# jzombie/rust-llkv

Hardware: NVIDIA B200
Metric: tpch_q6_lineitem_rows_per_sec (higher is better)
Workload: dtype i128/i64 (Decimal128, Date32)

## Files before the change

### rust-llkv_b200/csrc/compiler.cpp

```cpp
#include "compiler.h"

#include <algorithm>

#include <math.h>
#include <stdarg.h>
#include <stdio.h>
#include <stdlib.h>
#include <string.h>

#include <map>
#include <stdexcept>

namespace llkv {

typedef __int128 i128;
typedef unsigned __int128 u128;

namespace {

struct CompileError {
  int32_t code;
  std::string msg;
};

// ... 1683 lines not shown
    out_.fast = false;
    p.n_finstr = 0;
    if (!req_.no_fast) {
      const size_t lits_mark = lits_.size();
      if (lower_fast()) {
        out_.fast = true;
        bool checked = false;
        for (uint32_t i = 0; i < p.n_finstr; ++i) {
          const FInstr& fi = p.fcode[i];
          const uint32_t fb = fi.a & 0x7f;
          if ((fi.op == FO_OP_COL || fi.op == FO_OP_LIT || fi.op == FO_OP_TMP) && (fb == FB_ADD_CK || fb == FB_SUB_CK || fb == FB_MUL_CK)) checked = true;
        }
        out_.can_narrow_fail = checked;
        p.n_lits = (uint32_t)lits_.size();
        for (size_t i = 0; i < lits_.size(); ++i) p.lits[i] = lits_[i];
      } else {
        lits_.resize(lits_mark);
        p.n_finstr = 0;
      }
    }
  }

  struct Iv {
    bool known = false;
    i128 lo = 0, hi = 0;
    bool is_float = false;
  };
  static Iv iv_exact(i128 v) {
    Iv x;
    x.known = true;
// ... 66 lines not shown
    else if (verbose) fprintf(stderr, "[llkv] lean lowering gave up at compiler.cpp:%d\n", line);
    return false;
  }
  bool lower_fast() {
    Plan& p = out_.plan;
    if (wide_ || req_.bitmap_mode) return lf_fail(__LINE__);
    if (plan_cols_.empty()) return lf_fail(__LINE__);
    for (const ColumnMeta* c : plan_cols_) {
      if (c->load_kind == LK_D128 && !c->dec_fits_i64) return lf_fail(__LINE__);
    }
    std::vector<FInstr> f;
    std::vector<Sym> st;
    bool tmp_used[kFastTmps] = {false, false, false};
    int max_tmps = 0;
    bool ok = true;
    auto map_load = [&](uint8_t lk) -> uint32_t {
      switch (lk) {
        case LK_I32: case LK_D32: return LKF_4;
        case LK_I64: case LK_U64: case LK_F64: case LK_D64: return LKF_8;
        case LK_D128: return LKF_16;
        case LK_U8: return LKF_1;
        case LK_STR8: return LKF_S1;
        case LK_I8: return LKF_1S;
        case LK_I16: return LKF_2;
        case LK_U16: return LKF_2U;
        case LK_U32: return LKF_4U;
        case LK_F32: return LKF_4F;
        default: ok = false; return LKF_8;
      }
    };
    auto femit = [&](uint16_t op, uint32_t a, uint32_t b, uint32_t c) {
// ... 30 lines not shown
        if (i == keep || st[i].where != Sym::ACC) continue;
        int k = -1;
        for (int t = 0; t < kFastTmps; ++t)
          if (!tmp_used[t]) { k = t; break; }
        if (k < 0) { ok = false; return; }
        tmp_used[k] = true;
        if (k + 1 > max_tmps) max_tmps = k + 1;
        femit(FO_ST_TMP, (uint8_t)k, 0, 0);
        st[i].where = Sym::TMP;
        st[i].tmp = (uint8_t)k;
      }
    };
    auto load_acc = [&](size_t i) {
      if (st[i].where == Sym::ACC) return;
      spill_acc(i);
      if (st[i].where == Sym::COL) femit_load(FO_LD_COL, 2, st[i].col, map_load(st[i].load));
      else if (st[i].where == Sym::LIT) femit_load(FO_LD_LIT, 1, st[i].lit, 0);
      else {
        femit_load(FO_LD_TMP, 3, st[i].tmp, 0);
        tmp_used[st[i].tmp] = false;
      }
      st[i].where = Sym::ACC;
    };
    auto emit_binary = [&](uint8_t fb) {
      const size_t n = st.size();
      Sym& a = st[n - 2];
      Sym& b = st[n - 1];
      uint8_t rev = 0;
      const Sym* other;
      if (a.where == Sym::ACC) other = &b;
      else if (b.where == Sym::ACC) { other = &a; rev = FB_REV; }
      else { load_acc(n - 2); other = &b; }
      if (!ok) return;
      if (other->where == Sym::COL) femit(FO_OP_COL, fb | rev, map_load(other->load), other->col);
      else if (other->where == Sym::LIT) femit(FO_OP_LIT, fb | rev, 0, other->lit);
      else femit(FO_OP_TMP, fb | rev, other->tmp, 0);
      free_sym(*other);
    };
    auto fold_lit = [&](Sym& x, i128 v) {
      x.lit = add_lit((uint64_t)(u128)v, (uint64_t)((u128)v >> 64));
      x.iv = iv_exact(v);
    };

    if (p.n_fast_words > (uint32_t)kLeanMaxWords) return lf_fail(__LINE__);
    for (uint32_t w = 0; w < p.n_fast_words; ++w) p.fast[w].lean_width = p.fast[w].lean_rowrel = 0;
    auto lean_word = [&](uint32_t w, uint8_t width, bool rowrel) {
      if (w >= p.n_fast_words) { ok = false; return; }
      if (p.fast[w].lean_width && (p.fast[w].lean_rowrel != 0) != rowrel) width = 8, rowrel = false;
      if (width > p.fast[w].lean_width) p.fast[w].lean_width = width;
// ... 40 lines not shown
                  }
                  continue;
                }
                if (pr.op == OP_IN_D) {
                  const i128 v = (i128)(((u128)L.hi << 64) | (u128)L.lo);
                  if (!fits_i64(v)) {
                    if (c.load_kind == LK_D128) return lf_fail(__LINE__);
                    continue;
                  }
                }
                run.push_back(mk_lit_i((i128)(int64_t)L.lo));
              }
              if (c.load_kind == LK_D128 && !c.dec_fits_i64) return lf_fail(__LINE__);
              if (lits_.size() + run.size() + 1 > (size_t)kMaxLits) return lf_fail(__LINE__);
              const uint32_t first = run.empty() ? 0u : add_lit_run(run);
              femit(FO_LEAF, in.a, map_load(in.b), first);
              f.back().g = 3u;
              f.back().f = (uint32_t)run.size();
              f.back().e = push;
              i += conjunct ? 2 : 1;
              break;
            }
            if (pr.op == OP_PRED_F) {
              const bool f32 = c.load_kind == LK_F32;
              auto key = [&](double d) -> int64_t {
                if (f32) {
                  const float x = (float)d;
                  int32_t b;
                  memcpy(&b, &x, 4);
                  return (int64_t)(b ^ ((b >> 31) & INT32_MAX));
                }
// ... 74 lines not shown
                  if (uk != LLKV_BOUND_UNBOUNDED) {
                    const i128 v = lit_val(li);
                    if (uk == LLKV_BOUND_EXCLUDED) { if (v <= tmin) empty = true; else hi = v - 1; } else hi = v;
                  }
                }
                if (lo < tmin) lo = tmin;
                if (hi > tmax) hi = tmax;
                if (lo > hi) empty = true;
              }
              Lit a, b;
              if (empty) { a = mk_lit_i(1); b = mk_lit_i(0); }
              else { a = mk_lit_i(lo); b = mk_lit_i(hi); }
              std::vector<Lit> run = {a, b};
              if (lits_.size() + 2 > (size_t)kMaxLits) return lf_fail(__LINE__);
              const uint32_t first = add_lit_run(run);
              femit(FO_LEAF, in.a, map_load(in.b), first);
              f.back().g = uns ? 1u : 0u;
              if (c.load_kind == LK_STR8 || c.load_kind == LK_U8 || c.load_kind == LK_U64) f.back().g = 1u;
              f.back().e = push;
              i += conjunct ? 2 : 1;
              break;
            }
          }
          Sym x;
          x.where = Sym::COL;
          x.col = in.a;
          x.load = in.b;
          x.iv = column_interval(c);
          x.nm = c.nullable ? (1u << in.a) : 0u;
          st.push_back(x);
          break;
// ... 101 lines not shown
          const size_t n2 = st.size();
          uint32_t cmp = in.a;
          const Sym* other;
          if (st[n2 - 2].where == Sym::ACC) other = &st[n2 - 1];
          else if (st[n2 - 1].where == Sym::ACC) {
            static const uint8_t mirrored[6] = {LLKV_CMP_EQ, LLKV_CMP_NE, LLKV_CMP_GT, LLKV_CMP_GE, LLKV_CMP_LT, LLKV_CMP_LE};
            other = &st[n2 - 2];
            cmp = mirrored[cmp];
          } else {
            load_acc(n2 - 2);
            other = &st[n2 - 1];
          }
          if (!ok) return lf_fail(__LINE__);
          const uint32_t kind = in.op == OP_CMP_U ? 1u : in.op == OP_CMP_F ? 2u : 0u;
          const uint32_t nm = st[n2 - 1].nm | st[n2 - 2].nm;
          if (other->where == Sym::COL) femit(FO_CMP, cmp | (kind << 4), 0u | (map_load(other->load) << 8), other->col);
          else if (other->where == Sym::LIT) femit(FO_CMP, cmp | (kind << 4), 1u, other->lit);
          else femit(FO_CMP, cmp | (kind << 4), 2u, other->tmp);
          f.back().h = nm;
          free_sym(st[n2 - 1]);
          free_sym(st[n2 - 2]);
          st.pop_back();
          st.pop_back();
          ++mask_depth;
          break;
        }
        case OP_ISNULL: {
          if (i >= select_end_ || st.empty() || mask_depth >= 8) return lf_fail(__LINE__);
          const uint32_t nm = st.back().nm;
          free_sym(st.back());
          st.pop_back();
// ... 20 lines not shown
          if (mask_depth != 1) return lf_fail(__LINE__);
          femit(FO_MASK_FILTER, 0, 0, 0);
          mask_depth = 0;
          break;
        case OP_MVCC: femit(FO_MVCC, in.a, in.b, 0); break;
        case OP_SELECT_DONE: femit(FO_SELECT_DONE, 0, 0, 0); break;
        case OP_GROUP: {
          const int nk = in.a;
          if ((int)st.size() < nk) return lf_fail(__LINE__);
          for (int k = nk - 1; k >= 0; --k) {
            const Sym x = st.back();
            if (x.where != Sym::COL) return lf_fail(__LINE__);
            if (x.nm && (p.single_wide_key || !p.key_nullable[k])) return lf_fail(__LINE__);
            st.pop_back();
            p.key_col[k] = x.col;
            p.key_load[k] = (uint8_t)map_load(x.load);
          }
          femit(FO_GROUP, (uint8_t)nk, 0, 0);
          break;
        }
        case OP_AGG_COUNT_STAR: femit(FO_COUNT_STAR, 0, in.b, in.c); lean_word(in.b, 4, false); break;
        case OP_AGG_FIRSTROW: femit(FO_FIRSTROW, 0, in.b, in.c); lean_word(in.b, 4, true); break;
        case OP_AGG_COUNT: case OP_AGG_SUM_I: case OP_AGG_SUM_D: case OP_AGG_FSUM: case OP_AGG_MIN_I: case OP_AGG_MAX_I:
        case OP_AGG_MIN_F: case OP_AGG_MAX_F: case OP_AGG_FIRSTVALID: case OP_AGG_FIRSTNAN: case OP_AGG_MIN_D: case OP_AGG_MAX_D: {
          if (st.empty()) return lf_fail(__LINE__);
          uint8_t a = 0;
          uint16_t op;
          bool keep = (in.a & 1) != 0;
          uint8_t width = 8;
          bool rowrel = false;
          switch (in.op) {
// ... 101 lines not shown
```

### rust-llkv_b200/csrc/compiler.h

```cpp
#pragma once
#include <stdint.h>

#include <string>
#include <vector>

#include "../../include/llkv_gpu.h"
#include "plan.h"

namespace llkv {

struct ColumnMeta {
  uint64_t field_id = 0;
  int32_t type = 0;
  int precision = 0, scale = 0;
  bool nullable = false;
  uint8_t load_kind = 0;
  uint32_t elem_bytes = 0;
  uint32_t arrow_bytes = 0;
  const void* dev_values = nullptr;
  const unsigned char* dev_validity = nullptr;
  uint64_t n_rows = 0;
  bool dec_fits_i64 = true;
  uint64_t min_bits = 0, max_bits = 0;
  bool has_minmax = false;
  uint8_t max_strlen = 0;
  bool str_non_ascii = false;
  const std::vector<std::string>* dict_sorted = nullptr;
  uint64_t dict_epoch = 0;
};

inline void literal_bytes(const llkv_literal& l, const char** p, size_t* n) {
  if (l.precision == LLKV_LIT_STRING_BY_REF) {
    *p = reinterpret_cast<const char*>(static_cast<uintptr_t>(l.lo));
    *n = static_cast<size_t>(l.hi);
  } else {
// ... 86 lines not shown
```

### rust-llkv_b200/csrc/lean_kernel.cuh

```cuda
#pragma once
#include "device_util.cuh"
#include "plan.h"

namespace llkv {

#define LLKV_FULL 0xffffffffu
#define LLKV_SLOW_HERE (SLOW && has_slow)

__device__ __forceinline__ double lean_f64(i64 v) { return __longlong_as_double(v); }
__device__ __forceinline__ i64 lean_bits(double d) { return __double_as_longlong(d); }

constexpr u64 kSlotTableFull = 1ull << 63;
static __device__ __noinline__ u64 lean_global_slot_raw(u64* gkeys, u64 gcap, uint32_t n_keys, u64 K) {
  if (n_keys == 0) return 0;
  if (K == kEmptyKey) return gcap;
  const u64 mask = gcap - 1;
  u64 h = mix64(K) & mask;
  for (u64 i = 0; i <= mask; ++i) {
    u64 cur = gkeys[h];
    if (cur == K) return h;
    if (cur == kEmptyKey) {
      const u64 old = atomicCAS(&gkeys[h], kEmptyKey, K);
      if (old == kEmptyKey || old == K) return h;
    }
// ... 370 lines not shown
          } else {
            const u64 span = (u64)hi - (u64)lo;
#pragma unroll
            for (int r = 0; r < R; ++r) {
              const i64 b = reinterpret_cast<const i64*>(base)[r * NC + tid];
              m |= (unsigned)(((u64)(b ^ ((b >> 63) & 0x7fffffffffffffffll)) - (u64)lo) <= span) << r;
            }
          }
        } else if (in.b == LKF_4) {
          const uint32_t l = (uint32_t)(int)lo, span = (uint32_t)(int)hi - l;
#pragma unroll
          for (int r = 0; r < R; ++r) {
            const uint32_t v = reinterpret_cast<const uint32_t*>(base)[r * NC + tid];
            m |= (unsigned)((v - l) <= span) << r;
          }
        } else if ((in.b == LKF_8 || in.b == LKF_16) && in.g == 0) {
          const u64 span = (u64)hi - (u64)lo;
          const int stride = in.b == LKF_16 ? 2 : 1;
#pragma unroll
          for (int r = 0; r < R; ++r) {
            const u64 v = reinterpret_cast<const u64*>(base)[stride * (r * NC + tid)];
            m |= (unsigned)((v - (u64)lo) <= span) << r;
          }
        } else {
          i64 v[R];
          load_col(in.a, in.b, v);
          const u64 span = (u64)hi - (u64)lo;
#pragma unroll
          for (int r = 0; r < R; ++r) m |= (unsigned)(((u64)v[r] - (u64)lo) <= span) << r;
        }
// ... 999 lines not shown
```

### rust-llkv_b200/csrc/llkv_gpu.cu

```cuda
#include <cuda_runtime.h>
#include <dlfcn.h>
#include <math.h>
#include <stdarg.h>
#include <stdio.h>
#include <stdlib.h>
#include <string.h>

#include <algorithm>
#include <atomic>
#include <map>
#include <memory>
#include <mutex>
#include <string>
#include <deque>
#include <string_view>
#include <thread>
#include <unordered_map>
#include <vector>

#include "../../include/llkv_gpu.h"
#include "compiler.h"
#include "jit.h"
#include "plan.h"
#include "upload.h"
// ... 170 lines not shown
  for (u64 i = (u64)blockIdx.x * blockDim.x + threadIdx.x; i < n; i += (u64)gridDim.x * blockDim.x) {
    const ulonglong2 w = in[i];
    out[i] = w.x;
    b = b || (i64)w.y != ((i64)w.x >> 63);
  }
  if (b) atomicOr(bad, 1u);
}
__global__ void narrow_dec32_kernel(const ulonglong2* __restrict__ in, int* __restrict__ out, u64 n) {
  for (u64 i = (u64)blockIdx.x * blockDim.x + threadIdx.x; i < n; i += (u64)gridDim.x * blockDim.x) out[i] = (int)in[i].x;
}
__global__ void widen_dec32_kernel(const int* __restrict__ in, ulonglong2* __restrict__ out, u64 n) {
  for (u64 i = (u64)blockIdx.x * blockDim.x + threadIdx.x; i < n; i += (u64)gridDim.x * blockDim.x) {
    const i64 v = in[i];
    out[i] = make_ulonglong2((u64)v, (u64)(v >> 63));
  }
}
__global__ void widen_dec_kernel(const u64* __restrict__ in, ulonglong2* __restrict__ out, u64 n) {
  for (u64 i = (u64)blockIdx.x * blockDim.x + threadIdx.x; i < n; i += (u64)gridDim.x * blockDim.x) {
    const u64 v = in[i];
    out[i] = make_ulonglong2(v, (u64)((i64)v >> 63));
  }
}
__global__ void widen_str_kernel(const unsigned char* __restrict__ in, u64* __restrict__ out, u64 n) {
  for (u64 i = (u64)blockIdx.x * blockDim.x + threadIdx.x; i < n; i += (u64)gridDim.x * blockDim.x) out[i] = ((u64)in[i] << 56) | 1ull;
}
__global__ void or_bits_kernel(unsigned int* __restrict__ dst, u64 dst_off, const unsigned char* __restrict__ src, u64 n) {
  const u64 nw = (n + 31) / 32;
  for (u64 w = (u64)blockIdx.x * blockDim.x + threadIdx.x; w < nw; w += (u64)gridDim.x * blockDim.x) {
    unsigned int bits = 0;
    for (int b = 0; b < 4; ++b) {
// ... 476 lines not shown
  std::vector<NarrowChunk> narrow_chunks;
  uint64_t h2d_bytes = 0;
  unsigned int* d_perm = nullptr;
  uint64_t perm_chunk_rows = 0, perm_version = 0;
  bool sparse = false;
  void* pend_dst = nullptr;
  const void* pend_src = nullptr;
  uint64_t pend_bytes = 0;
  std::vector<void*> deferred_free;
  uint64_t version = 1;
  uint64_t zones_version = 0;
  u64* d_zones = nullptr;
  size_t d_zones_cap = 0;
  std::vector<u64> h_zones;
  uint32_t scans_unchanged = 0;
};

typedef std::shared_ptr<std::deque<std::string>> StringStore;
static void own_string_literal(llkv_literal& l, StringStore& store) {
  if (l.kind != LLKV_LIT_STRING || l.precision != LLKV_LIT_STRING_BY_REF) return;
  if (!store) store = std::make_shared<std::deque<std::string>>();
  store->emplace_back(reinterpret_cast<const char*>(static_cast<uintptr_t>(l.lo)), static_cast<size_t>(l.hi));
  l.lo = static_cast<uint64_t>(reinterpret_cast<uintptr_t>(store->back().data()));
}

struct llkv_gpu_program {
  uint64_t serial = 0;
  StringStore strings;
  std::vector<llkv_eval_op> ops;
  std::vector<llkv_literal> literals;
// ... 61 lines not shown
  bool lean_have[4] = {false, false, false, false};
  uint32_t lean_grid2[4] = {0, 0, 0, 0}, lean_ctas2[4] = {1, 1, 1, 1};
  uint32_t pk_parts = 0, pk_shift = 0, pk_slots = 0, pk_dense = 0, pk_key_bits = 0, pk_row_bits = 0, pk_n_ops = 0, pk_used_parts = 0;
  uint32_t pk_op_bits[8] = {0, 0, 0, 0, 0, 0, 0, 0};
  u64* part_out = nullptr;
  size_t part_out_elems = 0;
  uint32_t* part_cursor = nullptr;
  uint32_t* d_tile_list = nullptr;
  size_t tile_list_cap = 0;
  std::vector<uint32_t> h_tile_list;
  uint64_t tile_list_key = 0;
  uint64_t tile_list_total = 0;
  bool tile_list_use = false;
  uint64_t lean_sig = 0;
  uint32_t lean_jit_runs = 0;
  uint32_t* d_flags = nullptr;
  uint32_t* h_flags = nullptr;
  unsigned char* h_stage = nullptr;
  size_t h_stage_bytes = 0;
  bool prefetched = false;
  cudaEvent_t stage_ev = nullptr;
  Plan* d_plan = nullptr;
  Plan* h_plan = nullptr;
  CompileResult cr;
  PendingRun pending;
  bool reset_pending = false;
  uint64_t plan_epoch = 1;
  uint64_t exec_key = 0;
  uint32_t exec_same = 0;
  cudaGraphExec_t graph_exec = nullptr;
// ... 524 lines not shown
    case LK_I32: case LK_D32: zone_minmax_kernel<int, true, 1><<<blocks, 256, 0, s>>>((const int*)v, n, col->d_zones); break;
    case LK_I64: case LK_D64: zone_minmax_kernel<i64, true, 1><<<blocks, 256, 0, s>>>((const i64*)v, n, col->d_zones); break;
    case LK_U8: zone_minmax_kernel<unsigned char, false, 1><<<blocks, 256, 0, s>>>((const unsigned char*)v, n, col->d_zones); break;
    case LK_U16: zone_minmax_kernel<unsigned short, false, 1><<<blocks, 256, 0, s>>>((const unsigned short*)v, n, col->d_zones); break;
    case LK_U32: zone_minmax_kernel<unsigned int, false, 1><<<blocks, 256, 0, s>>>((const unsigned int*)v, n, col->d_zones); break;
    case LK_U64: zone_minmax_kernel<u64, false, 1><<<blocks, 256, 0, s>>>((const u64*)v, n, col->d_zones); break;
    default: return LLKV_OK;
  }
  CUDA_TRY(cudaGetLastError());
  col->h_zones.resize(2 * n_zones);
  CUDA_TRY(cudaMemcpyAsync(col->h_zones.data(), col->d_zones, n_zones * 16, cudaMemcpyDeviceToHost, s));
  CUDA_TRY(cudaStreamSynchronize(s));
  col->zones_version = col->version;
  *ok = true;
  return LLKV_OK;
}

static int32_t widen_decimal(llkv_gpu_column* col, uint64_t rows) {
  CUDA_TRY(cudaDeviceSynchronize());
  ulonglong2* wide = (ulonglong2*)col->landing;
  if (!wide || col->landing_cap < col->cap_rows) {
    if (wide) CUDA_TRY(cudaFree(wide));
    col->landing = nullptr;
    CUDA_TRY(cudaMalloc((void**)&wide, col->cap_rows * 16));
    CUDA_TRY(cudaMemset(wide, 0, col->cap_rows * 16));
    col->landing_cap = col->cap_rows;
  }
  if (rows) {
    if (col->load_kind == LK_D32) widen_dec32_kernel<<<1184, 256>>>((const int*)col->values, wide, rows);
    else widen_dec_kernel<<<1184, 256>>>((const u64*)col->values, wide, rows);
// ... 1044 lines not shown
extern "C" int32_t llkv_gpu_column_destroy(llkv_gpu_column* col) {
  if (!col) return LLKV_OK;
  llkv_gpu_ctx* c = col->ctx;
  CTX_LOCK(c);
  cudaSetDevice(c->device);
  col->pend_bytes = 0;
  drain_jobs(col);
  cudaDeviceSynchronize();
  c->columns.erase(col->lfid);
  ++c->state_epoch;
  for (auto& kv : c->mvcc)
    if (kv.second.created_by == col || kv.second.deleted_by == col) kv.second.created_by = kv.second.deleted_by = nullptr;
  for (void* p : col->deferred_free) cudaFree(p);
  if (col->landing) cudaFree(col->landing);
  if (col->narrow) cudaFree(col->narrow);
  if (col->values) cudaFree(col->values);
  if (col->validity) cudaFree(col->validity);
  if (col->dstats) cudaFree(col->dstats);
  if (col->d_zones) cudaFree(col->d_zones);
  if (col->d_perm) cudaFree(col->d_perm);
  if (col->d_fit) cudaFree(col->d_fit);
  delete col;
  return LLKV_OK;
}

extern "C" int32_t llkv_gpu_program_compile(llkv_gpu_ctx* ctx, const llkv_eval_op* ops, int32_t n_ops, const llkv_literal* literals,
                                             int32_t n_literals, const llkv_scalar_node* nodes, int32_t n_nodes,
                                             const int32_t* list_roots, int32_t n_list_roots, llkv_gpu_program** out) {
  (void)ctx;
  if (!out) return set_error(LLKV_ERR_INVALID_ARGUMENT, "NULL argument");
// ... 67 lines not shown
  for (auto& kv : ctx->columns)
    if (lfid_table(kv.second->lfid) == (table_id & 0xffffull) && kv.second->sparse) sparse_table = true;
  if (!sparse_table) return LLKV_OK;
  for (auto& kv : ctx->columns) {
    llkv_gpu_column* col = kv.second;
    if (lfid_table(col->lfid) != (table_id & 0xffffull) || col->n_rows == longest || col->type == LLKV_PT_UTF8) continue;
    int32_t rc;
    if ((rc = column_flush(col))) return rc;
    if (is_narrow_decimal(col) && (rc = widen_decimal(col, col->n_rows))) return rc;
    if ((rc = column_grow(col, longest)) || (rc = ensure_validity(col))) return rc;
    CUDA_TRY(cudaStreamSynchronize(ctx->copy_streams[(size_t)col->stream_index]));
    col->n_rows = longest;
    col->sparse = true;
    col->sealed = false;
    ++col->version;
    ++ctx->state_epoch;
  }
  return LLKV_OK;
}

static int32_t table_exists_bits(llkv_gpu_ctx* ctx, uint64_t table_id, const std::vector<llkv_gpu_column*>& handles, uint64_t rows,
                                 const unsigned char** out) {
  *out = nullptr;
  bool sparse_table = false;
  for (llkv_gpu_column* h : handles) sparse_table = sparse_table || h->sparse;
  if (!sparse_table) return LLKV_OK;
  auto it = ctx->mvcc.find(table_id);
  llkv_gpu_column* created = nullptr;
  for (llkv_gpu_column* h : handles)
    if ((h->lfid >> 48) == 2 ) created = h;
// ... 54 lines not shown
      int32_t rc = llkv_gpu_column_seal(col);
      if (rc) return rc;
    }
    ColumnMeta m;
    m.field_id = lfid_field(col->lfid) | ((col->lfid >> 48) << 48);
    m.type = col->type;
    m.precision = col->precision;
    m.scale = col->scale;
    m.nullable = col->validity != nullptr;
    m.load_kind = col->load_kind;
    m.elem_bytes = col->elem_bytes;
    if (col->type == LLKV_PT_UTF8) m.arrow_bytes = 4 + (uint32_t)(col->n_rows ? (col->hstats.data_bytes + col->n_rows - 1) / col->n_rows : 0);
    else m.arrow_bytes = (uint32_t)prim_type_width(col->type);
    m.dev_values = col->values;
    m.dev_validity = (const unsigned char*)col->validity;
    m.n_rows = col->n_rows;
    m.dec_fits_i64 = col->hstats.not_i64 == 0;
    const bool is_signed = col->type == LLKV_PT_INT8 || col->type == LLKV_PT_INT16 || col->type == LLKV_PT_INT32 ||
                           col->type == LLKV_PT_INT64 || col->type == LLKV_PT_DATE32 || col->type == LLKV_PT_DATE64;
    const bool is_unsigned = col->type == LLKV_PT_UINT8 || col->type == LLKV_PT_UINT16 || col->type == LLKV_PT_UINT32 ||
                             col->type == LLKV_PT_UINT64 || col->type == LLKV_PT_BOOLEAN;
    const bool dec_narrow = col->type == LLKV_PT_DECIMAL128 && col->hstats.not_i64 == 0;
    if ((is_signed || is_unsigned || dec_narrow) && col->n_rows && col->hstats.min_enc <= col->hstats.max_enc) {
      m.has_minmax = true;
      m.min_bits = (is_signed || dec_narrow) ? (col->hstats.min_enc ^ 0x8000000000000000ull) : col->hstats.min_enc;
      m.max_bits = (is_signed || dec_narrow) ? (col->hstats.max_enc ^ 0x8000000000000000ull) : col->hstats.max_enc;
    }
    m.max_strlen = (uint8_t)col->hstats.max_strlen;
    m.str_non_ascii = (col->hstats.bad_string & 2u) != 0;
    if (col->dict) {
// ... 864 lines not shown

static uint64_t request_signature(const llkv_gpu_ctx* ctx, const CompileRequest& req, const llkv_gpu_program* prog, bool force_wide,
                                  const unsigned char* exists_bits) {
  uint64_t h = 0xcbf29ce484222325ull;
  h = fnv_pod(h, exists_bits);
  for (const ColumnMeta& c : req.cols) {
    h = fnv_pod(h, c.field_id);
    h = fnv_pod(h, c.type);
    h = fnv_pod(h, c.precision);
    h = fnv_pod(h, c.scale);
    h = fnv_pod(h, c.nullable);
    h = fnv_pod(h, c.load_kind);
    h = fnv_pod(h, c.elem_bytes);
    h = fnv_pod(h, c.dev_values);
    h = fnv_pod(h, c.dev_validity);
    h = fnv_pod(h, c.n_rows);
    h = fnv_pod(h, c.dec_fits_i64);
    h = fnv_pod(h, c.has_minmax);
    h = fnv_pod(h, c.min_bits);
    h = fnv_pod(h, c.max_bits);
    h = fnv_pod(h, c.max_strlen);
    h = fnv_pod(h, c.str_non_ascii);
    h = fnv_pod(h, c.dict_epoch);
    h = fnv_pod(h, (uint64_t)(c.dict_sorted ? c.dict_sorted->size() + 1 : 0));
  }
  if (prog) {
    h = fnv1a(h, prog->ops.data(), prog->ops.size() * sizeof(llkv_eval_op));
    h = fnv1a(h, prog->literals.data(), prog->literals.size() * sizeof(llkv_literal));
    if (prog->strings)
      for (const std::string& x : *prog->strings) h = fnv1a(fnv_pod(h, x.size()), x.data(), x.size());
// ... 174 lines not shown
  CUDA_TRY(cudaMemcpyAsync(a->h_stage, a->gwords, wbytes, cudaMemcpyDeviceToHost, ctx->stream));
  if (kbytes) CUDA_TRY(cudaMemcpyAsync(a->h_stage + wbytes, a->gkeys, kbytes, cudaMemcpyDeviceToHost, ctx->stream));
  if (!a->stage_ev) CUDA_TRY(cudaEventCreateWithFlags(&a->stage_ev, cudaEventDisableTiming));
  CUDA_TRY(cudaEventRecord(a->stage_ev, ctx->stream));
  a->stage_ev_valid = true;
  a->prefetched = true;
  return LLKV_OK;
}

static int32_t agg_launch(llkv_gpu_agg* a, const llkv_gpu_program* prog, int apply_mvcc, uint64_t row_begin, uint64_t row_end,
                          bool force_wide) {
  llkv_gpu_ctx* ctx = a->ctx;
  CompileRequest req;
  std::vector<llkv_gpu_column*> handles;
  uint64_t table_rows = 0;
  int32_t rc = build_request(ctx, a->table_id, prog, apply_mvcc, req, handles, &table_rows);
  if (rc) return rc;
  if (row_end > table_rows) return set_error(LLKV_ERR_INVALID_ARGUMENT, "row_end %llu beyond the table's %llu rows", (unsigned long long)row_end, (unsigned long long)table_rows);
  if (ctx->nccl_comm && ctx->n_ranks > 1 && !a->keys.empty()) {
    bool changed = false;
    if ((rc = agree_dictionaries(ctx, a, handles, &changed))) return rc;
    if (changed) {
      req = CompileRequest();
      handles.clear();
      if ((rc = build_request(ctx, a->table_id, prog, apply_mvcc, req, handles, &table_rows))) return rc;
    }
    if ((rc = agree_key_stats(ctx, a, req))) return rc;
  }
  Plan& p = a->cr.plan;
  Geometry g;
  LeanPlan& lean = a->lean;
  uint32_t lean_ctas = 1;
  bool use_jit = false;
  const unsigned char* exists_bits = nullptr;
  if ((rc = table_exists_bits(ctx, a->table_id, handles, table_rows, &exists_bits))) return rc;
  const uint64_t sig = request_signature(ctx, req, prog, force_wide, exists_bits);
  if (!(a->lean_sig == sig && a->cr.fast && a->frozen)) {
    a->lean_sig = 0;
    a->lean_jit_runs = 0;
    a->lean_have[0] = a->lean_have[1] = a->lean_have[2] = a->lean_have[3] = false;
    req.specs = a->specs.data();
    req.n_aggs = (int32_t)a->specs.size();
    req.agg_nodes = a->nodes.data();
    req.n_agg_nodes = (int32_t)a->nodes.size();
    req.key_fields = a->keys;
    req.expr_mode = a->expr_mode;
    req.force_wide = force_wide || ctx->tune_force_wide == 1;
    req.no_fast = ctx->tune_force_wide != 0;
    if ((rc = compile_plan(req, a->cr))) return set_error(rc, "%s", a->cr.error.c_str());
    if ((rc = agg_freeze_layout(a, a->cr))) return rc;
    p.exists_bits = exists_bits;
    if (a->cr.fast) a->lean_sig = sig;
    else if ((rc = plan_geometry(ctx, p, a->cr.wide, false, row_begin, row_end, a->hint, g))) return rc;
  }
  p.exists_bits = exists_bits;
  if (a->cr.fast) {
    auto geometry = [&](int which) -> int32_t {
      if (a->lean_have[which]) return LLKV_OK;
      LeanTune tn = lean_tune(ctx);
      tn.interpreted = which == 0;
      tn.partition = which >= 2;
      if (which == 3) {
        tn.packed = true;
        tn.pack_key_bits = a->pk_key_bits;
        tn.pack_row_bits = a->pk_row_bits;
        tn.pack_parts = a->pk_parts;
        for (int j = 0; j < 8; ++j) tn.pack_op_bits[j] = a->pk_op_bits[j];
      }
      Geometry gg;
      uint32_t cc = 1;
      const uint64_t hint_eff = a->hint && a->observed_groups > a->hint ? a->observed_groups : a->hint;
      int32_t grc = lean_geometry(tn, p, row_begin, row_end, hint_eff, a->lean2[which], gg, &cc);
      if (grc) return grc;
      a->lean_grid2[which] = gg.grid;
      a->lean_ctas2[which] = cc;
      a->lean_have[which] = true;
      return LLKV_OK;
    };
    if ((rc = geometry(0))) return rc;
    if (ctx->jit_mode == 2) use_jit = true;
    else if (ctx->jit_mode == 1) {
      if (a->lean_jit_runs < 2) {
        const std::string key(reinterpret_cast<const char*>(&a->lean2[0].s), sizeof(LeanShape));
        a->lean_jit_runs = ++ctx->shape_runs[key];
      }
      use_jit = a->lean_jit_runs >= 2;
    }
    int which = use_jit ? 1 : 0;
    if (ctx->partition_mode && ctx->jit_mode && a->lean2[0].s.direct_global && partition_eligible(p)) {
      const u64 table_bytes = a->gcap * (8ull + 8ull * a->n_gwords);
      const bool big = table_bytes > (64ull << 20) && row_end - row_begin >= (4ull << 20);
      if ((big || ctx->partition_mode >= 2) && a->gcap >= 64) {
        PackedLayout L;
        bool packed = false;
        if (!ctx->no_packed && ctx->partition_mode != 3 && packed_layout(p, a->hint, a->gcap, ctx->partition_mode == 2, L)) {
          if (a->pk_parts != L.parts || a->pk_shift != L.shift || a->pk_slots != L.slots || a->pk_dense != L.dense || a->pk_key_bits != L.key_bits ||
              a->pk_row_bits != L.row_bits || a->pk_n_ops != L.n_ops || memcmp(a->pk_op_bits, L.op_bits, sizeof(L.op_bits)) != 0)
            a->lean_have[3] = false;
          a->pk_parts = L.parts;
// ... 200 lines not shown
    a->info.packed_tuples = 0;
  } else {
    a->info.partitions = 0;
    a->info.packed_tuples = 0;
  }
  a->info.tiles_pruned = 0;
  bool use_tile_list = false;
  if (a->cr.fast && ctx->prune_mode && row_end > row_begin) {
    struct PruneLeaf { llkv_gpu_column* col; i64 lo, hi; bool uns; };
    std::vector<PruneLeaf> leaves;
    uint64_t key = fnv_pod(fnv_pod(fnv_pod(fnv_pod(sig, p.tile_rows), row_begin), row_end), ctx->prune_mode);
    for (uint32_t i = 0; i < lean.s.n_code; ++i) {
      const FInstr& in = lean.s.code[i];
      if (in.op != FO_LEAF || in.e) continue;
      if (in.g >= 2) continue;
      llkv_gpu_column* col = nullptr;
      for (llkv_gpu_column* h : handles)
        if (h->values == lean.col_base[in.a]) col = h;
      if (!col) continue;
      const bool col_unsigned64 = col->type == LLKV_PT_UINT64;
      if (col_unsigned64 != (in.g != 0)) continue;
      leaves.push_back(PruneLeaf{col, (i64)lean.lits[in.c], (i64)lean.lits[in.c + 1], in.g != 0});
      key = fnv_pod(fnv_pod(key, col->version), (uint64_t)(uintptr_t)col);
    }
    bool wanted = !leaves.empty();
    if (wanted && ctx->prune_mode == 1) {
      bool settled = true;
      for (PruneLeaf& L : leaves) settled = settled && L.col->scans_unchanged >= 1;
      for (PruneLeaf& L : leaves) ++L.col->scans_unchanged;
      wanted = settled;
    }
    if (wanted && a->tile_list_key == key) {
      use_tile_list = a->tile_list_use;
    } else if (wanted) {
      const u64 T = p.tile_rows;
      const u64 n_zones = (table_rows + kZoneRows - 1) / kZoneRows;
      std::vector<uint8_t> zone_ok(n_zones, 1);
      bool any_map = false;
      for (PruneLeaf& L : leaves) {
        bool ok = false;
        if ((rc = ensure_zones(L.col, &ok))) return rc;
        if (!ok || L.col->h_zones.size() != 2 * n_zones) continue;
        any_map = true;
        const u64* z = L.col->h_zones.data();
// ... 20 lines not shown
      if (a->tile_list_use && kept) {
        if (a->tile_list_cap < kept) {
          if (a->d_tile_list) CUDA_TRY(cudaFree(a->d_tile_list));
          a->d_tile_list = nullptr;
          a->tile_list_cap = 0;
          CUDA_TRY(cudaMalloc((void**)&a->d_tile_list, kept * 4));
          a->tile_list_cap = kept;
        }
        CUDA_TRY(cudaMemcpyAsync(a->d_tile_list, a->h_tile_list.data(), kept * 4, cudaMemcpyHostToDevice, ctx->stream));
        CUDA_TRY(cudaStreamSynchronize(ctx->stream));
      }
      use_tile_list = a->tile_list_use;
    }
    if (use_tile_list) a->info.tiles_pruned = (uint32_t)(a->tile_list_total - a->h_tile_list.size());
  }
  a->pending.timed = ctx->timing;
  if (ctx->timing) CUDA_TRY(cudaEventRecord(ctx->ev0, ctx->stream));
  uint32_t launches = 0;
  a->info.used_jit_kernel = 0;
  lean.tile_list = nullptr;
  lean.s.use_tile_list = use_tile_list ? 1u : 0u;
  const u64 list_n = use_tile_list ? a->h_tile_list.size() : 0;
  const u64 tiles_per_launch = std::max<u64>(1, max_rows_per_launch / p.tile_rows);
  u64 list_pos = 0;
  for (u64 rb = row_begin; use_tile_list || rb < row_end || (rb == row_begin && launches == 0); rb += max_rows_per_launch) {
    u64 re = std::min<u64>(row_end, rb + max_rows_per_launch);
    u64 first_tile = rb / p.tile_rows;
    u64 n_tiles = re > rb ? (re + p.tile_rows - 1) / p.tile_rows - first_tile : 0;
    if (use_tile_list) {
      if (list_pos >= list_n) break;
// ... 1147 lines not shown
```

Measured before the change: 370.0 billion.

## Build cached narrow scan images of settled columns for lean scans

Once a sealed column has been scanned at least once without changing, a copy narrowed to the smallest integer width its min/max stats allow (1, 2 or 4 bytes) is materialized on the device. The lean plan is then recompiled so its loads read the image, cutting bytes read per row for columns like dates, quantities and decimals in the Q6 filter. The lean kernel gains a range-leaf path for the narrow load forms. The cost is a one-time conversion kernel and extra device memory per column, a second compile pass, and extra plumbing to keep JIT shape keys and zone pruning tied to the original columns.

```diff
diff --git a/rust-llkv_b200/csrc/compiler.cpp b/rust-llkv_b200/csrc/compiler.cpp
--- a/rust-llkv_b200/csrc/compiler.cpp
+++ b/rust-llkv_b200/csrc/compiler.cpp
@@ -1721,6 +1721,16 @@
         out_.can_narrow_fail = checked;
         p.n_lits = (uint32_t)lits_.size();
         for (size_t i = 0; i < lits_.size(); ++i) p.lits[i] = lits_[i];
+        phys = 0;
+        for (size_t i = 0; i < plan_cols_.size(); ++i) {
+          const ColumnMeta& c = *plan_cols_[i];
+          if (c.scan_values) {
+            p.cols[i].base = c.scan_values;
+            p.cols[i].elem_bytes = c.scan_bytes;
+          }
+          phys += p.cols[i].elem_bytes;
+        }
+        out_.physical_bytes_per_row = phys;
       } else {
         lits_.resize(lits_mark);
         p.n_finstr = 0;
@@ -1817,7 +1827,12 @@
     bool tmp_used[kFastTmps] = {false, false, false};
     int max_tmps = 0;
     bool ok = true;
-    auto map_load = [&](uint8_t lk) -> uint32_t {
+    auto map_load = [&](uint32_t col, uint8_t lk) -> uint32_t {
+      const ColumnMeta& c = *plan_cols_[col];
+      if (c.scan_values) {
+        if (lk != c.load_kind) ok = false;
+        lk = c.scan_load;
+      }
       switch (lk) {
         case LK_I32: case LK_D32: return LKF_4;
         case LK_I64: case LK_U64: case LK_F64: case LK_D64: return LKF_8;
@@ -1878,7 +1893,7 @@
     auto load_acc = [&](size_t i) {
       if (st[i].where == Sym::ACC) return;
       spill_acc(i);
-      if (st[i].where == Sym::COL) femit_load(FO_LD_COL, 2, st[i].col, map_load(st[i].load));
+      if (st[i].where == Sym::COL) femit_load(FO_LD_COL, 2, st[i].col, map_load(st[i].col, st[i].load));
       else if (st[i].where == Sym::LIT) femit_load(FO_LD_LIT, 1, st[i].lit, 0);
       else {
         femit_load(FO_LD_TMP, 3, st[i].tmp, 0);
@@ -1896,7 +1911,7 @@
       else if (b.where == Sym::ACC) { other = &a; rev = FB_REV; }
       else { load_acc(n - 2); other = &b; }
       if (!ok) return;
-      if (other->where == Sym::COL) femit(FO_OP_COL, fb | rev, map_load(other->load), other->col);
+      if (other->where == Sym::COL) femit(FO_OP_COL, fb | rev, map_load(other->col, other->load), other->col);
       else if (other->where == Sym::LIT) femit(FO_OP_LIT, fb | rev, 0, other->lit);
       else femit(FO_OP_TMP, fb | rev, other->tmp, 0);
       free_sym(*other);
@@ -1967,7 +1982,7 @@
               if (c.load_kind == LK_D128 && !c.dec_fits_i64) return lf_fail(__LINE__);
               if (lits_.size() + run.size() + 1 > (size_t)kMaxLits) return lf_fail(__LINE__);
               const uint32_t first = run.empty() ? 0u : add_lit_run(run);
-              femit(FO_LEAF, in.a, map_load(in.b), first);
+              femit(FO_LEAF, in.a, map_load(in.a, in.b), first);
               f.back().g = 3u;
               f.back().f = (uint32_t)run.size();
               f.back().e = push;
@@ -2072,7 +2087,13 @@
               std::vector<Lit> run = {a, b};
               if (lits_.size() + 2 > (size_t)kMaxLits) return lf_fail(__LINE__);
               const uint32_t first = add_lit_run(run);
-              femit(FO_LEAF, in.a, map_load(in.b), first);
+              const uint32_t form = map_load(in.a, in.b);
+              if (!empty && (form == LKF_4 || form == LKF_1S || form == LKF_2)) {
+                if (lo < INT32_MIN || hi > INT32_MAX) return lf_fail(__LINE__);
+              } else if (!empty && (form == LKF_1 || form == LKF_2U || form == LKF_4U)) {
+                if (lo < 0 || hi > (i128)UINT32_MAX) return lf_fail(__LINE__);
+              }
+              femit(FO_LEAF, in.a, form, first);
               f.back().g = uns ? 1u : 0u;
               if (c.load_kind == LK_STR8 || c.load_kind == LK_U8 || c.load_kind == LK_U64) f.back().g = 1u;
               f.back().e = push;
@@ -2204,7 +2225,7 @@
           if (!ok) return lf_fail(__LINE__);
           const uint32_t kind = in.op == OP_CMP_U ? 1u : in.op == OP_CMP_F ? 2u : 0u;
           const uint32_t nm = st[n2 - 1].nm | st[n2 - 2].nm;
-          if (other->where == Sym::COL) femit(FO_CMP, cmp | (kind << 4), 0u | (map_load(other->load) << 8), other->col);
+          if (other->where == Sym::COL) femit(FO_CMP, cmp | (kind << 4), 0u | (map_load(other->col, other->load) << 8), other->col);
           else if (other->where == Sym::LIT) femit(FO_CMP, cmp | (kind << 4), 1u, other->lit);
           else femit(FO_CMP, cmp | (kind << 4), 2u, other->tmp);
           f.back().h = nm;
@@ -2255,7 +2276,7 @@
             if (x.nm && (p.single_wide_key || !p.key_nullable[k])) return lf_fail(__LINE__);
             st.pop_back();
             p.key_col[k] = x.col;
-            p.key_load[k] = (uint8_t)map_load(x.load);
+            p.key_load[k] = (uint8_t)map_load(x.col, x.load);
           }
           femit(FO_GROUP, (uint8_t)nk, 0, 0);
           break;
diff --git a/rust-llkv_b200/csrc/compiler.h b/rust-llkv_b200/csrc/compiler.h
--- a/rust-llkv_b200/csrc/compiler.h
+++ b/rust-llkv_b200/csrc/compiler.h
@@ -19,6 +19,9 @@
   uint32_t arrow_bytes = 0;
   const void* dev_values = nullptr;
   const unsigned char* dev_validity = nullptr;
+  const void* scan_values = nullptr;
+  uint32_t scan_bytes = 0;
+  uint8_t scan_load = 0;
   uint64_t n_rows = 0;
   bool dec_fits_i64 = true;
   uint64_t min_bits = 0, max_bits = 0;
diff --git a/rust-llkv_b200/csrc/lean_kernel.cuh b/rust-llkv_b200/csrc/lean_kernel.cuh
--- a/rust-llkv_b200/csrc/lean_kernel.cuh
+++ b/rust-llkv_b200/csrc/lean_kernel.cuh
@@ -408,6 +408,12 @@
             const uint32_t v = reinterpret_cast<const uint32_t*>(base)[r * NC + tid];
             m |= (unsigned)((v - l) <= span) << r;
           }
+        } else if (in.b == LKF_1S || in.b == LKF_1 || in.b == LKF_2 || in.b == LKF_2U || in.b == LKF_4U) {
+          i64 v[R];
+          load_col(in.a, in.b, v);
+          const uint32_t l = (uint32_t)lo, span = (uint32_t)hi - l;
+#pragma unroll
+          for (int r = 0; r < R; ++r) m |= (unsigned)(((uint32_t)v[r] - l) <= span) << r;
         } else if ((in.b == LKF_8 || in.b == LKF_16) && in.g == 0) {
           const u64 span = (u64)hi - (u64)lo;
           const int stride = in.b == LKF_16 ? 2 : 1;
diff --git a/rust-llkv_b200/csrc/llkv_gpu.cu b/rust-llkv_b200/csrc/llkv_gpu.cu
--- a/rust-llkv_b200/csrc/llkv_gpu.cu
+++ b/rust-llkv_b200/csrc/llkv_gpu.cu
@@ -208,6 +208,10 @@
     const i64 v = in[i];
     out[i] = make_ulonglong2((u64)v, (u64)(v >> 63));
   }
+}
+template <class S, class D>
+__global__ void narrow_image_kernel(const S* __restrict__ in, D* __restrict__ out, u64 n) {
+  for (u64 i = (u64)blockIdx.x * blockDim.x + threadIdx.x; i < n; i += (u64)gridDim.x * blockDim.x) out[i] = (D)in[i];
 }
 __global__ void widen_dec_kernel(const u64* __restrict__ in, ulonglong2* __restrict__ out, u64 n) {
   for (u64 i = (u64)blockIdx.x * blockDim.x + threadIdx.x; i < n; i += (u64)gridDim.x * blockDim.x) {
@@ -714,6 +718,12 @@
   size_t d_zones_cap = 0;
   std::vector<u64> h_zones;
   uint32_t scans_unchanged = 0;
+  void* img = nullptr;
+  uint64_t img_cap_bytes = 0;
+  uint64_t img_version = 0;
+  const void* img_src = nullptr;
+  uint32_t img_bytes = 0;
+  uint8_t img_load = 0;
 };
 
 typedef std::shared_ptr<std::deque<std::string>> StringStore;
@@ -805,6 +815,7 @@
   bool tile_list_use = false;
   uint64_t lean_sig = 0;
   uint32_t lean_jit_runs = 0;
+  std::string jit_key;
   uint32_t* d_flags = nullptr;
   uint32_t* h_flags = nullptr;
   unsigned char* h_stage = nullptr;
@@ -1359,6 +1370,75 @@
   col->zones_version = col->version;
   *ok = true;
   return LLKV_OK;
+}
+
+static bool scan_image_form(const llkv_gpu_column* col, uint8_t* load, uint32_t* bytes) {
+  if ((col->lfid >> 48) != 0 || col->dict || !col->sealed || col->n_rows == 0 || col->hstats.min_enc > col->hstats.max_enc) return false;
+  bool is_signed;
+  switch (col->type) {
+    case LLKV_PT_INT8: case LLKV_PT_INT16: case LLKV_PT_INT32: case LLKV_PT_INT64: case LLKV_PT_DATE32: case LLKV_PT_DATE64: is_signed = true; break;
+    case LLKV_PT_UINT8: case LLKV_PT_UINT16: case LLKV_PT_UINT32: case LLKV_PT_UINT64: is_signed = false; break;
+    case LLKV_PT_DECIMAL128: if (!is_narrow_decimal(col)) return false; is_signed = true; break;
+    default: return false;
+  }
+  uint32_t b;
+  if (is_signed) {
+    const i64 lo = (i64)(col->hstats.min_enc ^ 0x8000000000000000ull), hi = (i64)(col->hstats.max_enc ^ 0x8000000000000000ull);
+    b = (lo >= INT8_MIN && hi <= INT8_MAX) ? 1 : (lo >= INT16_MIN && hi <= INT16_MAX) ? 2 : (lo >= INT32_MIN && hi <= INT32_MAX) ? 4 : 8;
+  } else {
+    const u64 hi = col->hstats.max_enc;
+    b = hi <= 0xffull ? 1 : hi <= 0xffffull ? 2 : hi <= 0xffffffffull ? 4 : 8;
+  }
+  if (b >= col->elem_bytes) return false;
+  *bytes = b;
+  *load = is_signed ? (b == 1 ? LK_I8 : b == 2 ? LK_I16 : LK_I32) : (b == 1 ? LK_U8 : b == 2 ? LK_U16 : LK_U32);
+  return true;
+}
+static bool scan_image_current(const llkv_gpu_column* col) {
+  return col->img && col->img_version == col->version && col->img_src == col->values && col->sealed;
+}
+
+static int32_t scan_image(llkv_gpu_column* col, cudaStream_t s, bool* built) {
+  *built = false;
+  uint8_t lk = 0;
+  uint32_t b = 0;
+  if (scan_image_current(col) || !scan_image_form(col, &lk, &b)) return LLKV_OK;
+  const u64 cap_rows = (col->n_rows + 2 * kPadRows - 1) / kPadRows * kPadRows;
+  const u64 rows = std::min<u64>(col->cap_rows, cap_rows);
+  if (col->img_cap_bytes < cap_rows * b) {
+    if (col->img) CUDA_TRY(cudaFree(col->img));
+    col->img = nullptr;
+    col->img_cap_bytes = 0;
+    CUDA_TRY(cudaMalloc(&col->img, cap_rows * b));
+    col->img_cap_bytes = cap_rows * b;
+  }
+  col->img_version = 0;
+  const unsigned blocks = (unsigned)std::min<u64>((rows + 255) / 256, 1184);
+  const void* v = col->values;
+  void* o = col->img;
+  switch (col->elem_bytes * 16 + b) {
+    case 2 * 16 + 1: narrow_image_kernel<<<blocks, 256, 0, s>>>((const unsigned short*)v, (unsigned char*)o, rows); break;
+    case 4 * 16 + 1: narrow_image_kernel<<<blocks, 256, 0, s>>>((const unsigned int*)v, (unsigned char*)o, rows); break;
+    case 4 * 16 + 2: narrow_image_kernel<<<blocks, 256, 0, s>>>((const unsigned int*)v, (unsigned short*)o, rows); break;
+    case 8 * 16 + 1: narrow_image_kernel<<<blocks, 256, 0, s>>>((const u64*)v, (unsigned char*)o, rows); break;
+    case 8 * 16 + 2: narrow_image_kernel<<<blocks, 256, 0, s>>>((const u64*)v, (unsigned short*)o, rows); break;
+    case 8 * 16 + 4: narrow_image_kernel<<<blocks, 256, 0, s>>>((const u64*)v, (unsigned int*)o, rows); break;
+    default: return set_error(LLKV_ERR_INTERNAL, "no scan image from %u to %u bytes per row", col->elem_bytes, b);
+  }
+  CUDA_TRY(cudaGetLastError());
+  if (rows < cap_rows) CUDA_TRY(cudaMemsetAsync((char*)o + rows * b, 0, (cap_rows - rows) * b, s));
+  col->img_version = col->version;
+  col->img_src = col->values;
+  col->img_bytes = b;
+  col->img_load = lk;
+  *built = true;
+  return LLKV_OK;
+}
+
+static llkv_gpu_column* plan_column(const std::vector<llkv_gpu_column*>& handles, const void* base) {
+  for (llkv_gpu_column* h : handles)
+    if (h->values == base || (h->img && h->img == base)) return h;
+  return nullptr;
 }
 
 static int32_t widen_decimal(llkv_gpu_column* col, uint64_t rows) {
@@ -2433,6 +2513,7 @@
   for (void* p : col->deferred_free) cudaFree(p);
   if (col->landing) cudaFree(col->landing);
   if (col->narrow) cudaFree(col->narrow);
+  if (col->img) cudaFree(col->img);
   if (col->values) cudaFree(col->values);
   if (col->validity) cudaFree(col->validity);
   if (col->dstats) cudaFree(col->dstats);
@@ -2530,6 +2611,7 @@
     col->sparse = true;
     col->sealed = false;
     ++col->version;
+    col->scans_unchanged = 0;
     ++ctx->state_epoch;
   }
   return LLKV_OK;
@@ -2614,6 +2696,11 @@
     else m.arrow_bytes = (uint32_t)prim_type_width(col->type);
     m.dev_values = col->values;
     m.dev_validity = (const unsigned char*)col->validity;
+    if (scan_image_current(col)) {
+      m.scan_values = col->img;
+      m.scan_bytes = col->img_bytes;
+      m.scan_load = col->img_load;
+    }
     m.n_rows = col->n_rows;
     m.dec_fits_i64 = col->hstats.not_i64 == 0;
     const bool is_signed = col->type == LLKV_PT_INT8 || col->type == LLKV_PT_INT16 || col->type == LLKV_PT_INT32 ||
@@ -3508,6 +3595,9 @@
     h = fnv_pod(h, c.elem_bytes);
     h = fnv_pod(h, c.dev_values);
     h = fnv_pod(h, c.dev_validity);
+    h = fnv_pod(h, c.scan_values);
+    h = fnv_pod(h, c.scan_bytes);
+    h = fnv_pod(h, c.scan_load);
     h = fnv_pod(h, c.n_rows);
     h = fnv_pod(h, c.dec_fits_i64);
     h = fnv_pod(h, c.has_minmax);
@@ -3712,49 +3802,74 @@
   CompileRequest req;
   std::vector<llkv_gpu_column*> handles;
   uint64_t table_rows = 0;
-  int32_t rc = build_request(ctx, a->table_id, prog, apply_mvcc, req, handles, &table_rows);
-  if (rc) return rc;
-  if (row_end > table_rows) return set_error(LLKV_ERR_INVALID_ARGUMENT, "row_end %llu beyond the table's %llu rows", (unsigned long long)row_end, (unsigned long long)table_rows);
-  if (ctx->nccl_comm && ctx->n_ranks > 1 && !a->keys.empty()) {
-    bool changed = false;
-    if ((rc = agree_dictionaries(ctx, a, handles, &changed))) return rc;
-    if (changed) {
-      req = CompileRequest();
-      handles.clear();
-      if ((rc = build_request(ctx, a->table_id, prog, apply_mvcc, req, handles, &table_rows))) return rc;
-    }
-    if ((rc = agree_key_stats(ctx, a, req))) return rc;
-  }
+  int32_t rc = LLKV_OK;
   Plan& p = a->cr.plan;
   Geometry g;
   LeanPlan& lean = a->lean;
   uint32_t lean_ctas = 1;
   bool use_jit = false;
   const unsigned char* exists_bits = nullptr;
-  if ((rc = table_exists_bits(ctx, a->table_id, handles, table_rows, &exists_bits))) return rc;
-  const uint64_t sig = request_signature(ctx, req, prog, force_wide, exists_bits);
-  if (!(a->lean_sig == sig && a->cr.fast && a->frozen)) {
-    a->lean_sig = 0;
-    a->lean_jit_runs = 0;
-    a->lean_have[0] = a->lean_have[1] = a->lean_have[2] = a->lean_have[3] = false;
-    req.specs = a->specs.data();
-    req.n_aggs = (int32_t)a->specs.size();
-    req.agg_nodes = a->nodes.data();
-    req.n_agg_nodes = (int32_t)a->nodes.size();
-    req.key_fields = a->keys;
-    req.expr_mode = a->expr_mode;
-    req.force_wide = force_wide || ctx->tune_force_wide == 1;
-    req.no_fast = ctx->tune_force_wide != 0;
-    if ((rc = compile_plan(req, a->cr))) return set_error(rc, "%s", a->cr.error.c_str());
-    if ((rc = agg_freeze_layout(a, a->cr))) return rc;
-    p.exists_bits = exists_bits;
-    if (a->cr.fast) a->lean_sig = sig;
-    else if ((rc = plan_geometry(ctx, p, a->cr.wide, false, row_begin, row_end, a->hint, g))) return rc;
+  uint64_t sig = 0;
+  const bool multi_keys = ctx->nccl_comm && ctx->n_ranks > 1 && !a->keys.empty();
+  auto is_key = [&](uint64_t field) { return std::find(a->keys.begin(), a->keys.end(), field) != a->keys.end(); };
+  auto fill_request = [&](CompileRequest& r) {
+    r.specs = a->specs.data();
+    r.n_aggs = (int32_t)a->specs.size();
+    r.agg_nodes = a->nodes.data();
+    r.n_agg_nodes = (int32_t)a->nodes.size();
+    r.key_fields = a->keys;
+    r.expr_mode = a->expr_mode;
+    r.force_wide = force_wide || ctx->tune_force_wide == 1;
+    r.no_fast = ctx->tune_force_wide != 0;
+  };
+  for (int pass = 0;; ++pass) {
+    req = CompileRequest();
+    handles.clear();
+    if ((rc = build_request(ctx, a->table_id, prog, apply_mvcc, req, handles, &table_rows))) return rc;
+    if (row_end > table_rows) return set_error(LLKV_ERR_INVALID_ARGUMENT, "row_end %llu beyond the table's %llu rows", (unsigned long long)row_end, (unsigned long long)table_rows);
+    if (multi_keys) {
+      bool changed = false;
+      if ((rc = agree_dictionaries(ctx, a, handles, &changed))) return rc;
+      if (changed) {
+        req = CompileRequest();
+        handles.clear();
+        if ((rc = build_request(ctx, a->table_id, prog, apply_mvcc, req, handles, &table_rows))) return rc;
+      }
+      if ((rc = agree_key_stats(ctx, a, req))) return rc;
+      for (ColumnMeta& c : req.cols)
+        if (is_key(c.field_id)) c.scan_values = nullptr;
+    }
+    if ((rc = table_exists_bits(ctx, a->table_id, handles, table_rows, &exists_bits))) return rc;
+    sig = request_signature(ctx, req, prog, force_wide, exists_bits);
+    if (!(a->lean_sig == sig && a->cr.fast && a->frozen)) {
+      a->lean_sig = 0;
+      a->lean_jit_runs = 0;
+      a->jit_key.clear();
+      a->lean_have[0] = a->lean_have[1] = a->lean_have[2] = a->lean_have[3] = false;
+      fill_request(req);
+      if ((rc = compile_plan(req, a->cr))) return set_error(rc, "%s", a->cr.error.c_str());
+      if ((rc = agg_freeze_layout(a, a->cr))) return rc;
+      p.exists_bits = exists_bits;
+      if (a->cr.fast) a->lean_sig = sig;
+      else if ((rc = plan_geometry(ctx, p, a->cr.wide, false, row_begin, row_end, a->hint, g))) return rc;
+    }
+    if (pass || !a->cr.fast || a->in_capture) break;
+    bool built = false;
+    for (uint32_t c = 0; c < p.n_cols; ++c) {
+      llkv_gpu_column* h = plan_column(handles, p.cols[c].base);
+      if (!h || h->scans_unchanged == 0 || (multi_keys && is_key(lfid_field(h->lfid)))) continue;
+      bool b = false;
+      if ((rc = scan_image(h, ctx->stream, &b))) return rc;
+      built = built || b;
+    }
+    if (!built) break;
   }
   p.exists_bits = exists_bits;
+  std::vector<llkv_gpu_column*> plan_handles;
+  if (a->cr.fast)
+    for (uint32_t c = 0; c < p.n_cols; ++c) plan_handles.push_back(plan_column(handles, p.cols[c].base));
   if (a->cr.fast) {
-    auto geometry = [&](int which) -> int32_t {
-      if (a->lean_have[which]) return LLKV_OK;
+    auto lean_geo = [&](int which, const Plan& plan, LeanPlan& lp, Geometry& gg, uint32_t* cc) -> int32_t {
       LeanTune tn = lean_tune(ctx);
       tn.interpreted = which == 0;
       tn.partition = which >= 2;
@@ -3765,10 +3880,14 @@
         tn.pack_parts = a->pk_parts;
         for (int j = 0; j < 8; ++j) tn.pack_op_bits[j] = a->pk_op_bits[j];
       }
+      const uint64_t hint_eff = a->hint && a->observed_groups > a->hint ? a->observed_groups : a->hint;
+      return lean_geometry(tn, plan, row_begin, row_end, hint_eff, lp, gg, cc);
+    };
+    auto geometry = [&](int which) -> int32_t {
+      if (a->lean_have[which]) return LLKV_OK;
       Geometry gg;
       uint32_t cc = 1;
-      const uint64_t hint_eff = a->hint && a->observed_groups > a->hint ? a->observed_groups : a->hint;
-      int32_t grc = lean_geometry(tn, p, row_begin, row_end, hint_eff, a->lean2[which], gg, &cc);
+      int32_t grc = lean_geo(which, p, a->lean2[which], gg, &cc);
       if (grc) return grc;
       a->lean_grid2[which] = gg.grid;
       a->lean_ctas2[which] = cc;
@@ -3779,8 +3898,31 @@
     if (ctx->jit_mode == 2) use_jit = true;
     else if (ctx->jit_mode == 1) {
       if (a->lean_jit_runs < 2) {
-        const std::string key(reinterpret_cast<const char*>(&a->lean2[0].s), sizeof(LeanShape));
-        a->lean_jit_runs = ++ctx->shape_runs[key];
+        if (a->jit_key.empty()) {
+          bool images = false;
+          for (const ColumnMeta& c : req.cols) images = images || c.scan_values;
+          if (!images) {
+            a->jit_key.assign(reinterpret_cast<const char*>(&a->lean2[0].s), sizeof(LeanShape));
+          } else {
+            CompileRequest r = req;
+            for (ColumnMeta& c : r.cols) c.scan_values = nullptr;
+            if (r.mvcc.enabled) {
+              r.mvcc.created_by = &r.cols[(size_t)(req.mvcc.created_by - req.cols.data())];
+              r.mvcc.deleted_by = &r.cols[(size_t)(req.mvcc.deleted_by - req.cols.data())];
+            }
+            fill_request(r);
+            std::unique_ptr<CompileResult> rcr(new CompileResult());
+            if ((rc = compile_plan(r, *rcr))) return set_error(rc, "%s", rcr->error.c_str());
+            if (!rcr->fast) return set_error(LLKV_ERR_INTERNAL, "a lean plan over scan images has no lean form over its resident columns");
+            rcr->plan.exists_bits = exists_bits;
+            std::unique_ptr<LeanPlan> lp(new LeanPlan());
+            Geometry gg;
+            uint32_t cc = 1;
+            if ((rc = lean_geo(0, rcr->plan, *lp, gg, &cc))) return rc;
+            a->jit_key.assign(reinterpret_cast<const char*>(&lp->s), sizeof(LeanShape));
+          }
+        }
+        a->lean_jit_runs = ++ctx->shape_runs[a->jit_key];
       }
       use_jit = a->lean_jit_runs >= 2;
     }
@@ -4011,9 +4153,7 @@
       const FInstr& in = lean.s.code[i];
       if (in.op != FO_LEAF || in.e) continue;
       if (in.g >= 2) continue;
-      llkv_gpu_column* col = nullptr;
-      for (llkv_gpu_column* h : handles)
-        if (h->values == lean.col_base[in.a]) col = h;
+      llkv_gpu_column* col = plan_handles[in.a];
       if (!col) continue;
       const bool col_unsigned64 = col->type == LLKV_PT_UINT64;
       if (col_unsigned64 != (in.g != 0)) continue;
@@ -4024,7 +4164,6 @@
     if (wanted && ctx->prune_mode == 1) {
       bool settled = true;
       for (PruneLeaf& L : leaves) settled = settled && L.col->scans_unchanged >= 1;
-      for (PruneLeaf& L : leaves) ++L.col->scans_unchanged;
       wanted = settled;
     }
     if (wanted && a->tile_list_key == key) {
@@ -4075,6 +4214,9 @@
     }
     if (use_tile_list) a->info.tiles_pruned = (uint32_t)(a->tile_list_total - a->h_tile_list.size());
   }
+  for (size_t c = 0; c < plan_handles.size() && !a->in_rerun; ++c)
+    if (plan_handles[c] && std::find(plan_handles.begin(), plan_handles.begin() + c, plan_handles[c]) == plan_handles.begin() + c)
+      ++plan_handles[c]->scans_unchanged;
   a->pending.timed = ctx->timing;
   if (ctx->timing) CUDA_TRY(cudaEventRecord(ctx->ev0, ctx->stream));
   uint32_t launches = 0;
```

Result: faster. 444.5 billion, median of 6 (+20.1%).
